# Luolin0826/band

Hardware: AMD Instinct MI355X
Metric: multi-DNN inferences/sec + p99 job latency, 4-model int8 mix @1/2/4/8 GPU (higher is better)
Workload: dtype int8

## Files before the change

### band_amd/_abi.py

```python
import ctypes
import os

_HERE = os.path.dirname(os.path.abspath(__file__))
LIB_PATH = os.path.join(_HERE, "libband_hip%s.so" % (
    "_" + os.environ["BAND_HIP_LIB_VARIANT"] if os.environ.get("BAND_HIP_LIB_VARIANT") else ""))

c_int, c_int32, c_void_p, c_size_t = ctypes.c_int, ctypes.c_int32, ctypes.c_void_p, ctypes.c_size_t


class ConvParams(ctypes.Structure):
    _fields_ = [(n, c_int) for n in (
        "batch", "in_h", "in_w", "in_c", "out_h", "out_w", "out_c", "k_h", "k_w",
        "stride_h", "stride_w", "dil_h", "dil_w", "pad_h", "pad_w", "k_pad", "n_pad", "in_xor")] + [
        (n, c_int32) for n in ("in_zp", "w_zp", "out_zp", "act_min", "act_max")] + [
        (n, c_void_p) for n in ("input", "output", "weights", "bias_eff", "mult", "shift", "residual")] + [
        (n, c_int32) for n in ("add_y_off", "add_r_off", "add_o_off", "add_left_shift", "add_y_mult",
                               "add_y_shift", "add_r_mult", "add_r_shift", "add_o_mult", "add_o_shift",
                               "add_act_min", "add_act_max")] + [("out_table", c_void_p), ("requant_fast", c_int32),
                                                                  ("kernel_hint", c_int32),
                                                                  ("out_img_stride", ctypes.c_int64)]


class ConvGroupedParams(ctypes.Structure):
    _fields_ = [("conv", ConvParams), ("groups", c_int32)]
# ... 62 lines not shown


class LayerNormParams(ctypes.Structure):
    _fields_ = [("rows", ctypes.c_long), ("depth", c_int), ("mean_x", MeanRowsParams), ("mean_d", MeanRowsParams)] + [
        (n, EltwiseParams) for n in ("sqdiff", "add_eps", "mul_gamma", "mul_x", "mul_m", "sub_beta", "add_out")] + [
        ("eps_q", c_int32)] + [(n, c_void_p) for n in ("rsqrt_table", "input", "gamma", "beta", "output")]


LAYERNORM_F32_MAX_DEPTH = 1024


class LayerNormF32Params(ctypes.Structure):
    _fields_ = [("rows", ctypes.c_long), ("depth", c_int), ("eps", ctypes.c_float)] + [
        (n, c_void_p) for n in ("input", "gamma", "beta", "output", "q", "scale", "offset")] + [("asymmetric", c_int)]


class DetectionParams(ctypes.Structure):
    _fields_ = [(n, c_int) for n in ("batch", "num_boxes", "num_classes", "num_classes_with_background",
                                     "max_detections")] + [
        (n, ctypes.c_float) for n in ("score_threshold", "iou_threshold", "scale_y", "scale_x", "scale_h",
                                      "scale_w")] + [
        ("box_type", c_int), ("score_type", c_int), ("box_scale", ctypes.c_float), ("score_scale", ctypes.c_float),
        ("box_zp", c_int32), ("score_zp", c_int32)] + [
        (n, c_void_p) for n in ("box_encodings", "class_scores", "anchors", "out_boxes", "out_classes",
                                "out_scores", "out_num", "scratch")]


class ChainParams(ctypes.Structure):
    _fields_ = [("dw", DwConvParams), ("pw1", ConvParams), ("pw2", ConvParams), ("has_pw2", c_int),
                ("px_blocks", c_int), ("waves", c_int), ("persist", c_int), ("tile", c_int),
                ("tile_blob", c_void_p), ("debug_stamps", c_void_p), ("deep", c_int), ("c_split", c_int),
                ("stage", c_int), ("dense", c_int)]


CONCAT_MAX_INPUTS = 16


class ConcatParams(ctypes.Structure):
    _fields_ = [("n_inputs", c_int), ("outer", ctypes.c_long),
                ("row", ctypes.c_long * CONCAT_MAX_INPUTS), ("input", c_void_p * CONCAT_MAX_INPUTS),
                ("table", c_void_p * CONCAT_MAX_INPUTS), ("output", c_void_p)]


class PadParams(ctypes.Structure):
    _fields_ = [("elem_bytes", c_int), ("in_shape", c_int * 4), ("pad_before", c_int * 4),
                ("pad_after", c_int * 4), ("value", ctypes.c_uint32), ("input", c_void_p), ("output", c_void_p),
                ("mode", c_int32)]


class ResizeNearestParams(ctypes.Structure):
    _fields_ = [(n, c_int) for n in ("batch", "in_h", "in_w", "out_h", "out_w", "row_bytes")] + [
        (n, c_void_p) for n in ("y_index", "x_index", "input", "output")]


class ResizeBilinearParams(ctypes.Structure):
    _fields_ = [(n, c_int) for n in ("batch", "in_h", "in_w", "channels", "out_h", "out_w")] + [
        (n, c_void_p) for n in ("y_tab", "x_tab", "input", "output")]


ARG_I8, ARG_U8, ARG_F32 = 0, 1, 2


class ArgMinMaxParams(ctypes.Structure):
    _fields_ = [(n, ctypes.c_long) for n in ("outer", "axis_len", "inner")] + [
        (n, c_int) for n in ("in_type", "is_min", "out_bytes")] + [("input", c_void_p), ("output", c_void_p)]

# ... 200 lines not shown
    "bh_dynquant_rows_check": (c_int, [ctypes.POINTER(DynQuantParams)]),
    "bh_fc_hybrid": (c_int, [ctypes.POINTER(FcHybridParams), c_void_p]),
    "bh_fc_hybrid_kernel": (ctypes.c_char_p, [ctypes.POINTER(FcHybridParams)]),
    "bh_fc_hybrid_check": (c_int, [ctypes.POINTER(FcHybridParams)]),
    "bh_dynquant_items": (c_int, [ctypes.POINTER(DynQuantItemsParams), c_void_p]),
    "bh_dynquant_items_kernel": (ctypes.c_char_p, [ctypes.POINTER(DynQuantItemsParams)]),
    "bh_dynquant_items_check": (c_int, [ctypes.POINTER(DynQuantItemsParams)]),
    "bh_conv2d_hybrid": (c_int, [ctypes.POINTER(ConvHybridParams), c_void_p]),
    "bh_conv2d_hybrid_kernel": (ctypes.c_char_p, [ctypes.POINTER(ConvHybridParams)]),
    "bh_conv2d_hybrid_check": (c_int, [ctypes.POINTER(ConvHybridParams)]),
    "bh_dwconv2d_hybrid": (c_int, [ctypes.POINTER(ConvHybridParams), c_void_p]),
    "bh_dwconv2d_hybrid_kernel": (ctypes.c_char_p, [ctypes.POINTER(ConvHybridParams)]),
    "bh_dwconv2d_hybrid_check": (c_int, [ctypes.POINTER(ConvHybridParams)]),
    "bh_softmax_i8": (c_int, [ctypes.POINTER(SoftmaxParams), c_void_p]),
    "bh_attention_i8": (c_int, [ctypes.POINTER(AttentionParams), c_void_p]),
    "bh_attention_i8_kernel": (ctypes.c_char_p, [ctypes.POINTER(AttentionParams)]),
    "bh_attention_i8_check": (c_int, [ctypes.POINTER(AttentionParams)]),
    "bh_attention_i8_lds_bytes": (c_size_t, [ctypes.POINTER(AttentionParams)]),
    "bh_zero_insert": (c_int, [ctypes.POINTER(ZeroInsertParams), c_void_p]),
    "bh_conv2d_f32": (c_int, [ctypes.POINTER(ConvF32Params), c_void_p]),
    "bh_conv2d_f32_split": (c_int, [ctypes.POINTER(ConvF32Params)]),
    "bh_fc_f32": (c_int, [ctypes.POINTER(FcF32Params), c_void_p]),
    "bh_eltwise_f32": (c_int, [ctypes.POINTER(EltwiseF32Params), c_void_p]),
    "bh_pool_f32": (c_int, [ctypes.POINTER(PoolF32Params), c_void_p]),
    "bh_unary_f32": (c_int, [c_int, c_void_p, c_void_p, ctypes.c_long, ctypes.c_float, ctypes.c_float, c_void_p]),
    "bh_softmax_f32": (c_int, [c_void_p, c_void_p, ctypes.c_long, c_int, ctypes.c_float, c_void_p]),
    "bh_dwconv2d_i8": (c_int, [ctypes.POINTER(DwConvParams), c_void_p]),
    "bh_fc_i8": (c_int, [ctypes.POINTER(FcParams), c_void_p]),
    "bh_eltwise_i8": (c_int, [ctypes.POINTER(EltwiseParams), c_void_p]),
    "bh_pool_i8": (c_int, [ctypes.POINTER(PoolParams), c_void_p]),
    "bh_irb_i8": (c_int, [ctypes.POINTER(IrbParams), c_void_p]),
    "bh_irb_lds_bytes": (c_size_t, [ctypes.POINTER(IrbParams)]),
    "bh_chain_i8": (c_int, [ctypes.POINTER(ChainParams), c_void_p]),
    "bh_mean": (c_int, [ctypes.POINTER(MeanParams), c_void_p]),
    "bh_mean_rows": (c_int, [ctypes.POINTER(MeanRowsParams), c_void_p]),
    "bh_mean_rows_kernel": (ctypes.c_char_p, [ctypes.POINTER(MeanRowsParams)]),
    "bh_mean_rows_check": (c_int, [ctypes.POINTER(MeanRowsParams)]),
    "bh_layernorm_i8": (c_int, [ctypes.POINTER(LayerNormParams), c_void_p]),
    "bh_layernorm_i8_kernel": (ctypes.c_char_p, [ctypes.POINTER(LayerNormParams)]),
    "bh_layernorm_i8_check": (c_int, [ctypes.POINTER(LayerNormParams)]),
    "bh_layernorm_f32": (c_int, [ctypes.POINTER(LayerNormF32Params), c_void_p]),
    "bh_layernorm_f32_kernel": (ctypes.c_char_p, [ctypes.POINTER(LayerNormF32Params)]),
    "bh_layernorm_f32_check": (c_int, [ctypes.POINTER(LayerNormF32Params)]),
    "bh_detection_scratch_bytes": (c_size_t, [c_int, c_int]),
    "bh_detection_postprocess": (c_int, [ctypes.POINTER(DetectionParams), c_void_p]),
    "bh_chain_lds_bytes": (c_size_t, [ctypes.POINTER(ChainParams)]),
    "bh_chain_tile_lds_bytes": (c_size_t, [ctypes.POINTER(ChainParams)]),
    "bh_chain_tile_launch": (c_int, [ctypes.POINTER(ChainParams), c_void_p]),
    "bh_chain_tile_blob_bytes": (c_size_t, [ctypes.POINTER(ChainParams)]),
    "bh_chain_tile_pack": (c_int, [ctypes.POINTER(ChainParams), c_void_p, c_void_p]),
    "bh_chain_stage_lds_bytes": (c_size_t, [ctypes.POINTER(ChainParams)]),
    "bh_chain_stage_launch": (c_int, [ctypes.POINTER(ChainParams), c_void_p]),
    "bh_chain_dense_lds_bytes": (c_size_t, [ctypes.POINTER(ChainParams)]),
    "bh_chain_dense_launch": (c_int, [ctypes.POINTER(ChainParams), c_void_p]),
    "bh_last_error": (ctypes.c_char_p, []),
}

BACKEND_SYMBOLS = {}

_lib = None
_configured = set()


class BandHipError(RuntimeError):
    pass

# ... 24 lines not shown
```

### band_amd/csrc/backend/hip/fusion.cc

```cpp
#include "backend/hip/chain_form.h"
#include "backend/hip/env.h"
#include "backend/hip/executor_internal.h"
#include <mutex>
#include <optional>
#include <unordered_map>

namespace band {
namespace hip {

using namespace ex;

namespace {
bool LaunchIo(const Launch& l, std::vector<const void*>* rd, std::vector<const void*>* wr) {
  switch (l.kind()) {
    case Launch::kConv:
    case Launch::kConvGrouped:
      *rd = {l.conv().input, l.conv().residual};
      *wr = {l.conv().output};
      return true;
    case Launch::kDwConv:
      *rd = {l.as<bh_dwconv_params>().input};
      *wr = {l.as<bh_dwconv_params>().output};
      return true;
    case Launch::kChain: {
// ... 514 lines not shown
    bh_chain_params& fc = F.Set<Launch::kChain>();
    F.op_index = D.op_index;
    if (form.launches == 0 || !instantiate(form, &fc)) {
      out.push_back(L[i]);
      continue;
    }
    if (fc.tile_blob) sg->consts.push_back(form.launches == 3 ? blob3 : blob2);
    const bool three = form.launches == 3;
    F.out_tensor = three ? P2->out_tensor : P1.out_tensor;
    F.kernel = fc.dense   ? "chain_dense_kernel"
               : fc.stage ? "chain_stage_kernel"
                          : (fc.tile ? "chain_tile_kernel" : "chain_kernel");
    const bh_dwconv_params& dw = fc.dw;
    const bh_conv_params& a = fc.pw1;
    const double px = static_cast<double>(dw.batch) * dw.out_h * dw.out_w;
    F.alg_bytes = static_cast<double>(dw.batch) * dw.in_h * dw.in_w * dw.in_c + 9.0 * dw.out_c + 28.0 * dw.out_c +
                  (a.residual ? px * a.out_c : 0.0) + (a.output ? px * a.out_c : 0.0) +
                  static_cast<double>(a.out_c) * a.in_c + 12.0 * a.out_c;
    F.alg_ops = D.alg_ops + P1.alg_ops;
    if (three) {
      const bh_conv_params& b = fc.pw2;
      F.alg_bytes += px * b.out_c + static_cast<double>(b.out_c) * b.in_c + 12.0 * b.out_c;
      F.alg_ops += P2->alg_ops;
      if (!a.output) sg->fused_tensors.insert(P1.out_tensor);
    }
    out.push_back(F);
    sg->fused_tensors.insert(D.out_tensor);
    i += three ? 2 : 1;
  }
  sg->launches.swap(out);
}

namespace {
void** OutSlot(Launch& l) {
  switch (l.kind()) {
    case Launch::kChain: {
      bh_chain_params& c = l.as<bh_chain_params>();
      return c.has_pw2 ? &c.pw2.output : &c.pw1.output;
    }
    case Launch::kConv:
    case Launch::kConvGrouped: return &l.conv().output;
    case Launch::kDwConv: return &l.as<bh_dwconv_params>().output;
    case Launch::kFc: return &l.as<bh_fc_params>().output;
    case Launch::kEltwise: return &l.as<bh_eltwise_params>().out;
    case Launch::kPool: return &l.as<bh_pool_params>().output;
    case Launch::kIrb: return &l.as<bh_irb_params>().output;
    case Launch::kLutU8: return &l.as<LutArgs>().dst;
    default: return nullptr;
  }
}
const void** TableSlot(Launch& l) {
  switch (l.kind()) {
    case Launch::kConv:
    case Launch::kConvGrouped: return l.conv().residual ? nullptr : &l.conv().out_table;
    case Launch::kDwConv: return &l.as<bh_dwconv_params>().out_table;
    case Launch::kFc: return &l.as<bh_fc_params>().out_table;
    default: return nullptr;
  }
}
}

void HipModelExecutor::FuseGlue(const HipModel& model, PreparedSubgraph* sg) {
  const TflModel& d = model.desc();
  auto private_chain = [&](int t, int to, std::vector<int>* chain) {
    while (t >= 0) {
      if (consumers_[t].size() != 1 || KeptOutside(d, *sg, t)) return false;
// ... 121 lines not shown
```

### band_amd/csrc/backend/hip/launch.h

```cpp
#pragma once

#include <cstddef>
#include <cstdint>
#include <cstdio>
#include <cstdlib>
#include <memory>
#include <type_traits>
#include <utility>
#include <variant>
#include <vector>

#include "backend/hip/cpu_kernels.h"
#include "band_hip_kernels.h"

namespace band {
namespace hip {

struct CopyArgs {
  void* dst;
  const void* src;
  size_t bytes;
};
struct LutArgs {
  const void* src;
// ... 117 lines not shown
      {kEltwiseF32, kIndex<bh_eltwise_f32_params>},
      {kPoolF32, kIndex<bh_pool_f32_params>},
      {kUnaryF32, kIndex<UnaryF32Args>},
      {kSoftmaxF32, kIndex<SoftmaxF32Args>},
      {kResizeBilinearU8, kIndex<bh_resize_bilinear_u8_params>},
      {kDetectionPost, kIndex<CpuDetectionParams>},
      {kMean, kIndex<bh_mean_params>},
      {kMeanRows, kIndex<bh_mean_rows_params>},
      {kConvGroup, kIndex<ConvGroupArgs>},
      {kDetectionGpu, kIndex<bh_detection_params>},
      {kArgMinMax, kIndex<bh_argminmax_params>},
      {kResizeArgMinMax, kIndex<bh_resize_argminmax_params>},
      {kReindex, kIndex<bh_reindex_params>},
      {kConvGrouped, kIndex<bh_conv_grouped_params>},
      {kBatchMatMul, kIndex<bh_batch_matmul_params>},
      {kBatchMatMulF32, kIndex<bh_batch_matmul_params>},
      {kLayerNorm, kIndex<LayerNormArgs>},
      {kAttention, kIndex<bh_attention_params>},
      {kDynQuantRows, kIndex<bh_dynquant_params>},
      {kFcHybrid, kIndex<bh_fc_hybrid_params>},
      {kDynQuantItems, kIndex<bh_dynquant_items_params>},
      {kConvHybrid, kIndex<bh_conv_hybrid_params>},
      {kDwConvHybrid, kIndex<bh_conv_hybrid_params>},
      {kLayerNormF32, kIndex<bh_layernorm_f32_params>},
  };
  template <Kind K>
  using PayloadOf = std::variant_alternative_t<kPayloads[K].index, Payload>;

  int op_index = -1;
  int out_tensor = -1;
  double alg_bytes = 0;
  double alg_ops = 0;
  const char* kernel = "";

  Kind kind() const { return kind_; }

  template <Kind K>
  PayloadOf<K>& Set(PayloadOf<K> p = {}) {
    kind_ = K;
    return payload_.template emplace<PayloadOf<K>>(std::move(p));
  }
  template <class P>
  P& Set(Kind k, P p) {
    if (k < 0 || k >= kNumKinds || kPayloads[k].index != kIndex<P>) Mismatch(k, kIndex<P>);
    kind_ = k;
    return payload_.template emplace<P>(std::move(p));
  }

  template <class P>
  P* get_if() { return std::get_if<P>(&payload_); }
  template <class P>
  const P* get_if() const { return std::get_if<P>(&payload_); }
  template <class P>
  P& as() {
    if (P* p = get_if<P>()) return *p;
    Mismatch(kind_, kIndex<P>);
  }
  template <class P>
  const P& as() const { return const_cast<Launch*>(this)->as<P>(); }

  bh_conv_params* conv_if() {
    if (bh_conv_grouped_params* g = get_if<bh_conv_grouped_params>()) return &g->conv;
    return get_if<bh_conv_params>();
  }
  const bh_conv_params* conv_if() const { return const_cast<Launch*>(this)->conv_if(); }
  bh_conv_params& conv() {
// ... 30 lines not shown
```

### band_amd/csrc/backend/hip/lower.cc

```cpp
#include "backend/hip/executor_internal.h"

namespace band {
namespace hip {

using namespace ex;

namespace {

struct ConvQuant {
  std::vector<int32_t> mult, shift;
  int32_t amin, amax, in_zp, w_zp;
  const int32_t* bias;
};

ConvQuant QuantOf(const TflModel& d, const ConvGeometry& g, const TflTensor& out) {
  const TflTensor& in = d.tensors[g.input];
  const TflTensor& w = d.tensors[g.filter];
  const bool i8 = in.type == DataType::kInt8;
  ConvQuant q;
  ConvMultipliers(Scale(in), w.scale, g.out_c, Scale(out), !i8, &q.mult, &q.shift);
  ActivationRangeQuantized(g.act, Scale(out), Zp(out), i8, &q.amin, &q.amax);
  q.in_zp = Dom(in);
  q.w_zp = i8 ? 0 : Dom(w);
  q.bias = g.bias >= 0 ? reinterpret_cast<const int32_t*>(d.tensors[g.bias].data) : nullptr;
// ... 380 lines not shown
        bh_resize_bilinear_params& p = L->Set<Launch::kResizeBilinear>();
        p.batch = b; p.in_h = ih; p.in_w = iw; p.channels = c; p.out_h = oh; p.out_w = ow;
        p.y_tab = static_cast<const int32_t*>(dt);
        p.x_tab = static_cast<const int32_t*>(dt) + 3 * oh;
        p.input = in_ptr;
        p.output = out_ptr;
        L->kernel = "resize_bilinear_kernel";
      }
      return absl::OkStatus();
    }
    default:
      return absl::InternalError(std::string("no lowering for ") + TflBuiltinName(op.builtin));
  }
}

absl::Status HipModelExecutor::BuildLaunches(const HipModel& model, PreparedSubgraph* sg) {
  sg->launches.clear();
  sg->fused_ops.clear();
  sg->fused_tensors.clear();
  for (int i : sg->ops) {
    if (sg->fused_ops.count(i)) continue;
    RETURN_STATUS_IF(Lower(model, i, sg));
  }
  if (opt_.allow_fusion && opt_.allow_chain && device_flag_ == DeviceFlag::kGPU) FuseChains(model, sg);
  if (opt_.allow_fusion && opt_.allow_irb && device_flag_ == DeviceFlag::kGPU) FuseBlocks(model, sg);
  if (opt_.allow_fusion && opt_.allow_layernorm && device_flag_ == DeviceFlag::kGPU) FuseLayerNorm(model, sg);
  if (opt_.allow_fusion && opt_.allow_layernorm && opt_.fused_layernorm_f32 && device_flag_ == DeviceFlag::kGPU) {
    FuseLayerNormF32(model, sg);
    FoldLayerNormQuant(model, sg);
  }
  if (opt_.allow_fusion && opt_.fused_attention && device_flag_ == DeviceFlag::kGPU) FuseAttention(model, sg);
  if (opt_.allow_fusion) FuseGlue(model, sg);
  if (opt_.allow_fusion && opt_.allow_group && device_flag_ == DeviceFlag::kGPU) RETURN_STATUS_IF(GroupConvs(sg));
  return absl::OkStatus();
}

bool HipModelExecutor::TryFuseResidualAdd(const HipModel& model, int oi, PreparedSubgraph* sg, Launch* L) {
  if (!opt_.allow_fusion || !opt_.allow_add) return false;
  const TflModel& d = model.desc();
  const int t = d.ops[oi].outputs[0];
  if (consumers_[t].size() != 1) return false;
  const int j = consumers_[t][0];
  if (j <= oi || !std::binary_search(sg->ops.begin(), sg->ops.end(), j)) return false;
  const TflOperator& add = d.ops[j];
  if ((add.builtin != kTflAdd && add.builtin != kTflSub) || add.inputs.size() != 2) return false;
  if (!GpuSupports(d, add, nullptr)) return false;
  if (KeptOutside(d, *sg, t)) return false;
  const bool conv_is_first = add.inputs[0] == t;
  const int other = conv_is_first ? add.inputs[1] : add.inputs[0];
  if (other == t) return false;
  if (other < 0 || producer_[other] > oi) return false;
  const TflTensor& tc = d.tensors[t];
  const TflTensor& tr = d.tensors[other];
  const TflTensor& to = d.tensors[add.outputs[0]];
  if (tr.shape != tc.shape || to.shape != tc.shape || tr.type != tc.type || to.type != tc.type) return false;
  void* rptr = nullptr;
  void* optr = nullptr;
  if (!DevicePtr(model, other, sg, &rptr).ok() || !DevicePtr(model, add.outputs[0], sg, &optr).ok()) return false;
  const TflTensor& t1 = d.tensors[add.inputs[0]];
  const TflTensor& t2 = d.tensors[add.inputs[1]];
  const AddParams ap = AddSubParams(Scale(t1), Scale(t2), Scale(to), add.builtin == kTflSub);
  bh_conv_params& p = L->conv();
  p.residual = rptr;
  p.output = optr;
  p.add_left_shift = ap.left_shift;
  p.add_y_off = -Zp(tc);
// ... 791 lines not shown
```

### band_amd/csrc/backend/hip/model_executor.cc

```cpp
#include "backend/hip/model_executor.h"

#include <sys/prctl.h>
#include <time.h>

#include <chrono>
#include <limits>
#include <mutex>
#include <unordered_map>

#include "backend/hip/affinity.h"
#include "backend/hip/completion.h"
#include "backend/hip/env.h"
#include "backend/hip/executor_internal.h"

namespace band {
namespace hip {

using namespace ex;

namespace ex {
thread_local bool t_variant_ctor = false;
}


// ... 7 lines not shown
    stream_ = DeviceRegistry::Get().StreamForWorker(worker_id_);
  } else if (device_flag_ == DeviceFlag::kCPU && !t_variant_ctor) {
    cpu_pool_ = std::make_shared<CpuPool>(num_threads_ > 0 ? num_threads_ : 1, PinnableCpus(thread_affinity_mask_));
  }
  use_graph_ = env::Graph();
  const std::string m(env::Sync());
  sync_mode_ = m == "block"    ? kSyncBlock
               : m == "poll"     ? kSyncPoll
               : m == "poller"   ? kSyncPoller
               : m == "spin"     ? kSyncSpin
                                 : kSyncAdaptive;
  block_sync_ = sync_mode_ == kSyncBlock;
  direct_io_ = env::DirectIo();
  coalesce_max_ = env::Coalesce();
  coalesce_lanes_ = env::CoalesceLanes();
  opt_.Latch(false);
}

void ExecOptions::Latch(bool bound) {
  if (!bound) {
    gpu_detection = env::GpuDetection();
    hybrid_conv = env::HybridConv();
  }
  if (!bound || latched) return;
  latched = true;
  const char* f = env::Fusion();
  if (f[0] == '0') allow_fusion = false;
  if (std::strcmp(f, "noirb") == 0) allow_irb = false;
  if (std::strcmp(f, "noadd") == 0) allow_add = false;
  if (std::strcmp(f, "nochain") == 0) allow_chain = false;
  if (std::strcmp(f, "nogroup") == 0) allow_group = false;
  if (std::strcmp(f, "noargmax") == 0) allow_argmax = false;
  if (std::strcmp(f, "nolayernorm") == 0) allow_layernorm = false;
  if (std::strcmp(f, "forcechain") == 0) forced_chain = ForcedChain::kPlain;
  if (std::strcmp(f, "forcetile") == 0) forced_chain = ForcedChain::kTile;
  if (std::strcmp(f, "forcedeep") == 0) forced_chain = ForcedChain::kDeep;
  if (std::strcmp(f, "forcestage") == 0) forced_chain = ForcedChain::kStage;
  if (std::strcmp(f, "forcedense") == 0) forced_chain = ForcedChain::kDense;
  if (std::strcmp(f, "notile") == 0) no_tile_chain = true;
  if (std::strcmp(f, "nodeep") == 0) no_deep_chain = true;
  if (std::strcmp(f, "nosplit") == 0) no_split_chain = true;
  if (std::strcmp(f, "nostage") == 0) no_stage_chain = true;
  autotune = env::Autotune();
  fused_attention = env::FusedAttention();
  fused_layernorm_f32 = env::FusedLayerNormF32();
}

HipModelExecutor::~HipModelExecutor() {
  if (coalescer_) coalescer_->Leave(this);
  coalescer_.reset();
  job_batches_.clear();
  if (ordinal_ >= 0) {
    bh_set_device(ordinal_);
    if (stream_) bh_stream_sync(stream_);
    for (auto& kv : subgraphs_) DropGraph(kv.second.get());
    if (done_event_) bh_event_destroy(done_event_);
  }
  subgraphs_.clear();
  if (owned_stream_) bh_stream_destroy(owned_stream_);
}

std::unique_ptr<HipModelExecutor> HipModelExecutor::MakeLane() {
  if (device_flag_ != DeviceFlag::kGPU || ordinal_ < 0) return nullptr;
  auto lane = std::make_unique<HipModelExecutor>(model_id_, worker_id_, device_flag_, thread_affinity_mask_,
                                                 num_threads_);
  if (bh_set_device(ordinal_) != 0 || bh_stream_create(&lane->owned_stream_) != 0) return nullptr;
// ... 486 lines not shown
  return std::make_shared<HipTensorView>(m, nullptr);
}

namespace {

struct KindCalls {
  Launch::Kind kind;
  int (*device)(const Launch&, bh_stream_t);
  void (*host)(const Launch&, CpuPool&);
};

template <class F>
struct BlockOf;
template <class R, class P, class... A>
struct BlockOf<R (*)(const P*, A...)> {
  using type = P;
};
template <class R, class P, class... A>
struct BlockOf<R (*)(const P&, A...)> {
  using type = P;
};
template <auto Fn>
int Dev(const Launch& l, bh_stream_t s) {
  return Fn(&l.as<typename BlockOf<decltype(Fn)>::type>(), s);
}
template <auto Fn>
void Host(const Launch& l, CpuPool& pool) {
  const auto& p = l.as<typename BlockOf<decltype(Fn)>::type>();
  if constexpr (std::is_invocable_v<decltype(Fn), decltype(p), CpuPool&>) Fn(p, pool);
  else Fn(p);
}

constexpr KindCalls kCalls[] = {
    {Launch::kConv, Dev<bh_conv2d_i8>, Host<CpuConv>},
    {Launch::kDwConv, Dev<bh_dwconv2d_i8>, Host<CpuDwConv>},
    {Launch::kFc, Dev<bh_fc_i8>, Host<CpuFc>},
    {Launch::kEltwise, Dev<bh_eltwise_i8>, Host<CpuEltwise>},
    {Launch::kPool, Dev<bh_pool_i8>, Host<CpuPool2D>},
    {Launch::kCopy,
     [](const Launch& l, bh_stream_t s) {
       const CopyArgs& c = l.as<CopyArgs>();
       return c.src != c.dst ? bh_copy_d2d(c.dst, c.src, c.bytes, s) : 0;
     },
     [](const Launch& l, CpuPool&) {
       const CopyArgs& c = l.as<CopyArgs>();
       if (c.src != c.dst) std::memmove(c.dst, c.src, c.bytes);
     }},
    {Launch::kIrb, Dev<bh_irb_i8>, nullptr},
    {Launch::kChain, Dev<bh_chain_i8>, nullptr},
    {Launch::kLutU8,
     [](const Launch& l, bh_stream_t s) {
       const LutArgs& a = l.as<LutArgs>();
       return bh_lut_u8(a.src, a.dst, a.count, a.table, s);
     },
     [](const Launch& l, CpuPool& pool) {
       const LutArgs& a = l.as<LutArgs>();
       CpuLutU8(a.src, a.dst, a.count, static_cast<const uint8_t*>(a.table), pool);
     }},
    {Launch::kLutF32,
     [](const Launch& l, bh_stream_t s) {
       const LutArgs& a = l.as<LutArgs>();
       return bh_lut_f32(a.src, a.dst, a.count, static_cast<const float*>(a.table), s);
     },
     [](const Launch& l, CpuPool& pool) {
       const LutArgs& a = l.as<LutArgs>();
       CpuLutF32(a.src, static_cast<float*>(a.dst), a.count, static_cast<const float*>(a.table), pool);
     }},
// ... 401 lines not shown
```

### band_amd/csrc/backend/hip/model_executor.h

```cpp
#pragma once

#include <functional>
#include <map>
#include <memory>
#include <set>
#include <string>
#include <vector>

#include "backend/hip/chain_form.h"
#include "backend/hip/coalescer.h"
#include "backend/hip/cpu_kernels.h"
#include "backend/hip/device.h"
#include "backend/hip/model.h"
#include "backend/hip/tensor.h"
#include "backend/hip/job_batching.h"
#include "backend/hip/launch.h"
#include "backend/hip/lower_args.h"
#include "band/interface/model_executor.h"
#include "band_hip_kernels.h"

namespace band {
namespace hip {

struct LnMatch;
// ... 10 lines not shown
  std::vector<int> ops;
  std::vector<int> inputs, outputs;
  bool model_order_io = false;
  std::map<int, size_t> offset;
  std::shared_ptr<DeviceBlob> arena;
  std::map<int, std::unique_ptr<PinnedBuffer>> host;
  std::set<int> extra_d2h;
  std::set<int> fused_ops;
  std::set<int> fused_tensors;
  std::set<int> no_fuse;
  std::vector<Launch> launches;
  std::vector<std::shared_ptr<DeviceBlob>> consts;
  bh_graph_exec_t graph = nullptr;
  bool io_in_graph = true;
  void* graph_tmpl = nullptr;
  struct IoNode {
    void* node;
    int tensor;
    bool h2d;
  };
  std::vector<IoNode> io_nodes;
  bool io_retargeted = false;
  int runs = 0;
  double wait_us = 0.0;
};

struct ExecOptions {
  bool allow_fusion = true;
  bool allow_irb = true, allow_add = true;
  bool allow_chain = true;
  bool allow_group = true;
  bool allow_argmax = true;
  bool allow_layernorm = true;
  ForcedChain forced_chain = ForcedChain::kNone;
  bool no_tile_chain = false;
  bool no_deep_chain = false;
  bool no_split_chain = false;
  bool no_stage_chain = false;
  bool autotune = true;
  bool gpu_detection = false;
  bool hybrid_conv = false;
  bool fused_attention = false;
  bool fused_layernorm_f32 = false;
  bool latched = false;
  void Latch(bool bound);
};

class HipModelExecutor : public interface::IModelExecutor, public IJobBatching {
 public:
  HipModelExecutor(ModelId model_id, WorkerId worker_id, DeviceFlag device_flag,
                   CpuSet thread_affinity_mask, int num_threads);
  ~HipModelExecutor() override;

  absl::StatusOr<ModelSpec> InvestigateModelSpec(interface::IModel* model) override;
  absl::Status PrepareSubgraph(interface::IModel* model, std::set<int> ops = {},
                               std::set<int> unit_indices = {}) override;
  BackendType GetBackendType() const override { return BackendType::kTfLite; }
  const std::vector<int>& GetInputs(const SubgraphKey& key) const override;
  const std::vector<int>& GetOutputs(const SubgraphKey& key) const override;
  const char* GetInputName(const SubgraphKey& key, int index) const override;
  const char* GetOutputName(const SubgraphKey& key, int index) const override;
  size_t GetNumTensors(const SubgraphKey& key) const override;
  size_t GetNumNodes(const SubgraphKey& key) const override;
  std::shared_ptr<interface::ITensorView> GetTensorView(const SubgraphKey& key, int index) override;
  bool HasSubgraph(const SubgraphKey& key) const override;
  SubgraphKey GetLargestSubgraphKey() const override;
// ... 7 lines not shown
  absl::Status ExecuteJobBatch(const SubgraphKey& key, int n) override;
  absl::Status ExecuteJobBatchDirect(const SubgraphKey& key, int n, const std::vector<const interface::ITensor*>& in,
                                     const std::vector<interface::ITensor*>& out) override;

  void SetUseGraph(bool on) { use_graph_ = on; }
  absl::Status ProfileSubgraph(const SubgraphKey& key, int iters, std::vector<OpTiming>* out,
                               double* floor_us = nullptr);
  absl::Status LaunchKernels(const SubgraphKey& key, std::vector<const char*>* out) const;
  absl::Status JobBatchLaunchKernels(const SubgraphKey& key, int n, std::vector<const char*>* out) const;
  absl::Status TimeSubgraph(const SubgraphKey& key, int iters, double* us);
  int ordinal() const { return ordinal_; }
  const JobCoalescer* coalescer() const { return coalescer_.get(); }

  static bool GpuSupports(const TflModel& model, const TflOperator& op, std::string* why);
  static bool CpuSupports(const TflModel& model, const TflOperator& op, std::string* why);
  bool GpuSupportsHere(const TflModel& model, const TflOperator& op, std::string* why) const;
  bool CpuSupportsHere(const TflModel& model, const TflOperator& op, std::string* why) const;

 private:
  friend class JobCoalescer;
  PreparedSubgraph* Find(const SubgraphKey& key) const;
  absl::Status RunPass(PreparedSubgraph* sg);
  std::unique_ptr<HipModelExecutor> MakeLane();
  absl::Status EnsureMeta(const HipModel& model);
  absl::Status Lower(const HipModel& model, int op_index, PreparedSubgraph* sg);
  absl::Status BuildLaunches(const HipModel& model, PreparedSubgraph* sg);
  bool TryFuseResidualAdd(const HipModel& model, int conv_op, PreparedSubgraph* sg, Launch* l);
  void FuseBlocks(const HipModel& model, PreparedSubgraph* sg);
  bool PackChainTile(bh_chain_params* q, std::shared_ptr<DeviceBlob>* blob);
  bool KeptOutside(const TflModel& d, const PreparedSubgraph& sg, int t) const;
  bool PrivateTensor(const TflModel& d, const PreparedSubgraph& sg, int t, int only_consumer) const;
  bool PrivateTo(const TflModel& d, const PreparedSubgraph& sg, int t, const std::set<int>& ops) const;
  void FuseChains(const HipModel& model, PreparedSubgraph* sg);
  void FuseGlue(const HipModel& model, PreparedSubgraph* sg);
  bool MatchLayerNorm(const TflModel& d, const PreparedSubgraph& sg, const std::vector<Launch>& ls, size_t i,
                      const Launch::Kind kinds[10], LnMatch* n) const;
  void FuseTenOps(const TflModel& d, PreparedSubgraph* sg, const Launch::Kind kinds[10],
                  const std::function<bool(const LnMatch& n, const Launch* l, Launch* F)>& fill);
  void FuseLayerNorm(const HipModel& model, PreparedSubgraph* sg);
  void FuseLayerNormF32(const HipModel& model, PreparedSubgraph* sg);
  void FoldLayerNormQuant(const HipModel& model, PreparedSubgraph* sg);
  void FuseAttention(const HipModel& model, PreparedSubgraph* sg);
  absl::Status GroupConvs(PreparedSubgraph* sg);
  double TimeLaunches(const std::vector<const Launch*>& ls, int iters);
  absl::Status DevicePtr(const HipModel& model, int tensor, PreparedSubgraph* sg, void** ptr);
  absl::Status ConstBlob(const std::string& key, size_t bytes, PreparedSubgraph* sg,
                         const std::function<absl::Status(uint8_t*)>& fill, std::shared_ptr<DeviceBlob>* blob);
  absl::Status UploadConst(const std::string& key, const void* data, size_t bytes, PreparedSubgraph* sg,
                           const void** dev);
  absl::Status LowerConv(const HipModel& model, int op_index, void* in_ptr, void* out_ptr, const std::string& ckey,
                         PreparedSubgraph* sg, Launch* l);
  absl::Status PackedConv(const HipModel& model, int op_index, const ex::ConvGeometry& g, bool flip,
                          const void* in_ptr, void* out_ptr, const std::string& ckey, PreparedSubgraph* sg, Launch* l);
  absl::Status LowerDepthwise(const HipModel& model, int op_index, void* in_ptr, void* out_ptr,
                              const std::string& ckey, PreparedSubgraph* sg, Launch* l);
  absl::Status LowerFc(const HipModel& model, int op_index, void* in_ptr, void* out_ptr, const std::string& ckey,
                       PreparedSubgraph* sg, Launch* l);
  absl::Status LowerFcHybrid(const HipModel& model, int op_index, void* in_ptr, void* out_ptr, const std::string& ckey,
                             PreparedSubgraph* sg, Launch* l);
  absl::Status LowerConvHybrid(const HipModel& model, int op_index, void* in_ptr, void* out_ptr, const std::string& ckey,
                               PreparedSubgraph* sg, Launch* l);
  absl::Status LowerEltwise(const HipModel& model, int op_index, void* in_ptr, void* out_ptr, PreparedSubgraph* sg,
                            Launch* l);
  absl::Status LowerPool(const HipModel& model, int op_index, void* in_ptr, void* out_ptr, Launch* l);
  absl::Status LowerMean(const HipModel& model, int op_index, void* in_ptr, void* out_ptr, Launch* l);
  absl::Status LowerArgMinMax(const HipModel& model, int op_index, void* in_ptr, void* out_ptr, Launch* l);
// ... 70 lines not shown
```

### include/band_hip_kernels.h

```cpp
#ifndef BAND_HIP_KERNELS_H_
#define BAND_HIP_KERNELS_H_

#include <stddef.h>
#include <stdint.h>

#ifdef __cplusplus
extern "C" {
#endif

#define BH_EINVAL (-1)

typedef void* bh_stream_t;
typedef void* bh_graph_exec_t;
typedef void* bh_event_t;

int bh_device_count(int* count);
int bh_set_device(int ordinal);
int bh_get_device(int* ordinal);
int bh_device_arch(int ordinal, char* buf, size_t cap);
int bh_device_pci_bus_id(int ordinal, char* buf, int cap);
int bh_stream_create(bh_stream_t* stream);
int bh_stream_destroy(bh_stream_t stream);
int bh_stream_sync(bh_stream_t stream);
int bh_stream_query(bh_stream_t stream);
// ... 173 lines not shown
  int32_t d_zp, d_act_min, d_act_max;
  const int8_t* proj_w; int proj_k_pad;
  const int32_t* proj_bias_eff; const int32_t* proj_mult; const int32_t* proj_shift;
  int32_t p_zp, p_act_min, p_act_max;
  int has_residual;
  int32_t add_p_off, add_x_off, add_o_off, add_left_shift;
  int32_t add_p_mult, add_p_shift, add_x_mult, add_x_shift, add_o_mult, add_o_shift;
  int32_t add_act_min, add_act_max;
  const void* input;
  void* output;
  void* debug_stamps;
  int32_t requant_fast;
} bh_irb_params;

size_t bh_irb_lds_bytes(const bh_irb_params* p);
int bh_irb_i8(const bh_irb_params* p, bh_stream_t s);

typedef struct bh_chain_params {
  bh_dwconv_params dw;
  bh_conv_params pw1;
  bh_conv_params pw2;
  int has_pw2;
  int px_blocks;
  int waves;
  int persist;
  int tile;
  const void* tile_blob;
  void* debug_stamps;
  int deep;
  int c_split;
  int stage;
  int dense;
} bh_chain_params;

size_t bh_chain_lds_bytes(const bh_chain_params* p);
size_t bh_chain_stage_lds_bytes(const bh_chain_params* p);
int bh_chain_stage_launch(const bh_chain_params* p, bh_stream_t s);
size_t bh_chain_dense_lds_bytes(const bh_chain_params* p);
int bh_chain_dense_launch(const bh_chain_params* p, bh_stream_t s);
size_t bh_chain_tile_lds_bytes(const bh_chain_params* p);
int bh_chain_tile_launch(const bh_chain_params* p, bh_stream_t s);
size_t bh_chain_tile_blob_bytes(const bh_chain_params* p);
int bh_chain_tile_pack(const bh_chain_params* p, void* blob, bh_stream_t s);
int bh_chain_i8(const bh_chain_params* p, bh_stream_t s);

typedef struct bh_mean_params {
  long outer, reduce, inner;
  int type;
  int32_t multiplier, shift, bias;
  const void* input;
  void* output;
} bh_mean_params;
int bh_mean(const bh_mean_params* p, bh_stream_t s);

typedef struct bh_mean_rows_params {
  long rows;
  int depth;
  int type;
  int exact;
  float scale, bias;
  int32_t out_zp;
  const void* input;
  void* output;
} bh_mean_rows_params;
int bh_mean_rows(const bh_mean_rows_params* p, bh_stream_t s);
const char* bh_mean_rows_kernel(const bh_mean_rows_params* p);
// ... 384 lines not shown
```

Measured before the change: 124,200.

## Fuse 1x1 conv with following 3x3 depthwise conv into one LDS-resident kernel

Adds a new HIP kernel that computes a 1x1 int8 pointwise conv via MFMA for whole small images, keeps the requantized result tile in LDS, and runs the 3x3 depthwise conv from LDS before writing only the final output. A fusion pass pairs adjacent conv/dwconv launches whose intermediate tensor is private, autotunes among four tile forms against the unfused pair, and caches the choice. This removes the intermediate tensor's global write and read plus one kernel launch for small spatial maps, at the cost of a BM-limited tiling (whole images per tile) and extra autotune time at preparation.

```diff
diff --git a/band_amd/_abi.py b/band_amd/_abi.py
--- a/band_amd/_abi.py
+++ b/band_amd/_abi.py
@@ -118,6 +118,12 @@
                 ("tile_blob", c_void_p), ("debug_stamps", c_void_p), ("deep", c_int), ("c_split", c_int),
                 ("stage", c_int), ("dense", c_int)]
 
+
+class ConvDwParams(ctypes.Structure):
+    _fields_ = [("pw", ConvParams), ("dw", DwConvParams), ("form", c_int)]
+
+
+CONV_DW_128, CONV_DW_64, CONV_DW_32, CONV_DW_64W8 = 1, 2, 3, 4
 
 CONCAT_MAX_INPUTS = 16
 
@@ -384,6 +390,10 @@
     "bh_irb_i8": (c_int, [ctypes.POINTER(IrbParams), c_void_p]),
     "bh_irb_lds_bytes": (c_size_t, [ctypes.POINTER(IrbParams)]),
     "bh_chain_i8": (c_int, [ctypes.POINTER(ChainParams), c_void_p]),
+    "bh_conv_dw": (c_int, [ctypes.POINTER(ConvDwParams), c_void_p]),
+    "bh_conv_dw_ok": (c_int, [ctypes.POINTER(ConvParams), ctypes.POINTER(DwConvParams)]),
+    "bh_conv_dw_images_per_tile": (c_int, [c_int, c_int]),
+    "bh_conv_dw_kernel": (ctypes.c_char_p, [ctypes.POINTER(ConvDwParams)]),
     "bh_mean": (c_int, [ctypes.POINTER(MeanParams), c_void_p]),
     "bh_mean_rows": (c_int, [ctypes.POINTER(MeanRowsParams), c_void_p]),
     "bh_mean_rows_kernel": (ctypes.c_char_p, [ctypes.POINTER(MeanRowsParams)]),
diff --git a/band_amd/csrc/backend/hip/fusion.cc b/band_amd/csrc/backend/hip/fusion.cc
--- a/band_amd/csrc/backend/hip/fusion.cc
+++ b/band_amd/csrc/backend/hip/fusion.cc
@@ -570,6 +570,69 @@
 }
 
 namespace {
+constexpr int kConvDwTuneVersion = 1;
+}
+
+void HipModelExecutor::FuseConvDw(const HipModel& model, PreparedSubgraph* sg) {
+  const TflModel& d = model.desc();
+  std::vector<Launch> out;
+  const auto& L = sg->launches;
+  for (size_t i = 0; i < L.size(); ++i) {
+    const bool pair = L[i].kind() == Launch::kConv && i + 1 < L.size() && L[i + 1].kind() == Launch::kDwConv &&
+                      bh_conv_dw_ok(&L[i].as<bh_conv_params>(), &L[i + 1].as<bh_dwconv_params>()) != 0 &&
+                      PrivateTensor(d, *sg, L[i].out_tensor, L[i + 1].op_index);
+    if (!pair) {
+      out.push_back(L[i]);
+      continue;
+    }
+    const Launch& P = L[i];
+    const Launch& D = L[i + 1];
+    bh_conv_dw_params q{};
+    q.pw = P.as<bh_conv_params>();
+    q.dw = D.as<bh_dwconv_params>();
+    const int by_shape = bh_conv_dw_ok(&q.pw, &q.dw);
+    char key[256];
+    std::snprintf(key, sizeof(key), "cd%d:%d:%d:%dx%dx%d:%d:s%dd%d:t%d%d", kConvDwTuneVersion, ordinal_,
+                  tune_batch_ > 0 ? tune_batch_ : q.pw.batch, q.pw.in_h, q.pw.in_w, q.pw.in_c, q.pw.out_c,
+                  q.dw.stride_h, q.dw.dil_h, q.pw.out_table ? 1 : 0, q.dw.taps ? 1 : 0);
+    const std::optional<int> cached = opt_.autotune && !opt_.force_conv_dw ? TuneLookup(key) : std::nullopt;
+    int form = 0;
+    if (opt_.force_conv_dw) {
+      form = by_shape;
+    } else if (cached) {
+      form = *cached >= 0 && *cached <= BH_CONV_DW_64W8 ? *cached : 0;
+    } else {
+      Fastest best(opt_.autotune ? TimeLaunches({&P, &D}, 10) : -1.0);
+      const bool measured = best.us > 0;
+      for (int f = BH_CONV_DW_128; measured && f <= BH_CONV_DW_64W8; ++f) {
+        if ((f == BH_CONV_DW_128 && q.pw.out_c <= 64) || (f != BH_CONV_DW_128 && f != BH_CONV_DW_32 && q.pw.out_c <= 32)) continue;
+        q.form = f;
+        Launch F = P;
+        F.conv_dw = std::make_shared<const bh_conv_dw_params>(q);
+        if (best.Offer(TimeLaunches({&F}, 10))) form = f;
+      }
+      if (measured) TuneStore(key, form);
+    }
+    if (form == 0) {
+      out.push_back(L[i]);
+      continue;
+    }
+    q.form = form;
+    Launch F = P;
+    F.conv_dw = std::make_shared<const bh_conv_dw_params>(q);
+    F.out_tensor = D.out_tensor;
+    F.kernel = "conv_dw_kernel";
+    const double mid = static_cast<double>(q.pw.batch) * q.pw.out_h * q.pw.out_w * q.pw.out_c;
+    F.alg_bytes = P.alg_bytes + D.alg_bytes - 2.0 * mid;
+    F.alg_ops = P.alg_ops + D.alg_ops;
+    out.push_back(F);
+    sg->fused_tensors.insert(P.out_tensor);
+    ++i;
+  }
+  sg->launches.swap(out);
+}
+
+namespace {
 void** OutSlot(Launch& l) {
   switch (l.kind()) {
     case Launch::kChain: {
diff --git a/band_amd/csrc/backend/hip/launch.h b/band_amd/csrc/backend/hip/launch.h
--- a/band_amd/csrc/backend/hip/launch.h
+++ b/band_amd/csrc/backend/hip/launch.h
@@ -173,6 +173,7 @@
   double alg_bytes = 0;
   double alg_ops = 0;
   const char* kernel = "";
+  std::shared_ptr<const bh_conv_dw_params> conv_dw;
 
   Kind kind() const { return kind_; }
 
diff --git a/band_amd/csrc/backend/hip/lower.cc b/band_amd/csrc/backend/hip/lower.cc
--- a/band_amd/csrc/backend/hip/lower.cc
+++ b/band_amd/csrc/backend/hip/lower.cc
@@ -436,6 +436,7 @@
   if (opt_.allow_fusion && opt_.fused_attention && device_flag_ == DeviceFlag::kGPU) FuseAttention(model, sg);
   if (opt_.allow_fusion) FuseGlue(model, sg);
   if (opt_.allow_fusion && opt_.allow_group && device_flag_ == DeviceFlag::kGPU) RETURN_STATUS_IF(GroupConvs(sg));
+  if (opt_.allow_fusion && opt_.allow_conv_dw && device_flag_ == DeviceFlag::kGPU) FuseConvDw(model, sg);
   return absl::OkStatus();
 }
 
diff --git a/band_amd/csrc/backend/hip/model_executor.cc b/band_amd/csrc/backend/hip/model_executor.cc
--- a/band_amd/csrc/backend/hip/model_executor.cc
+++ b/band_amd/csrc/backend/hip/model_executor.cc
@@ -63,6 +63,8 @@
   if (std::strcmp(f, "nogroup") == 0) allow_group = false;
   if (std::strcmp(f, "noargmax") == 0) allow_argmax = false;
   if (std::strcmp(f, "nolayernorm") == 0) allow_layernorm = false;
+  if (std::strcmp(f, "noconvdw") == 0) allow_conv_dw = false;
+  if (std::strcmp(f, "forceconvdw") == 0) force_conv_dw = true;
   if (std::strcmp(f, "forcechain") == 0) forced_chain = ForcedChain::kPlain;
   if (std::strcmp(f, "forcetile") == 0) forced_chain = ForcedChain::kTile;
   if (std::strcmp(f, "forcedeep") == 0) forced_chain = ForcedChain::kDeep;
@@ -615,7 +617,11 @@
 }
 
 constexpr KindCalls kCalls[] = {
-    {Launch::kConv, Dev<bh_conv2d_i8>, Host<CpuConv>},
+    {Launch::kConv,
+     [](const Launch& l, bh_stream_t s) {
+       return l.conv_dw ? bh_conv_dw(l.conv_dw.get(), s) : bh_conv2d_i8(&l.as<bh_conv_params>(), s);
+     },
+     Host<CpuConv>},
     {Launch::kDwConv, Dev<bh_dwconv2d_i8>, Host<CpuDwConv>},
     {Launch::kFc, Dev<bh_fc_i8>, Host<CpuFc>},
     {Launch::kEltwise, Dev<bh_eltwise_i8>, Host<CpuEltwise>},
diff --git a/band_amd/csrc/backend/hip/model_executor.h b/band_amd/csrc/backend/hip/model_executor.h
--- a/band_amd/csrc/backend/hip/model_executor.h
+++ b/band_amd/csrc/backend/hip/model_executor.h
@@ -66,6 +66,8 @@
   bool allow_group = true;
   bool allow_argmax = true;
   bool allow_layernorm = true;
+  bool allow_conv_dw = true;
+  bool force_conv_dw = false;
   ForcedChain forced_chain = ForcedChain::kNone;
   bool no_tile_chain = false;
   bool no_deep_chain = false;
@@ -139,6 +141,7 @@
   bool PrivateTensor(const TflModel& d, const PreparedSubgraph& sg, int t, int only_consumer) const;
   bool PrivateTo(const TflModel& d, const PreparedSubgraph& sg, int t, const std::set<int>& ops) const;
   void FuseChains(const HipModel& model, PreparedSubgraph* sg);
+  void FuseConvDw(const HipModel& model, PreparedSubgraph* sg);
   void FuseGlue(const HipModel& model, PreparedSubgraph* sg);
   bool MatchLayerNorm(const TflModel& d, const PreparedSubgraph& sg, const std::vector<Launch>& ls, size_t i,
                       const Launch::Kind kinds[10], LnMatch* n) const;
diff --git a/band_amd/csrc/kernels/conv_dw.hip b/band_amd/csrc/kernels/conv_dw.hip
--- /dev/null
+++ b/band_amd/csrc/kernels/conv_dw.hip
@@ -0,0 +1,312 @@
+#include "common.hpp"
+#include "conv_epilogue.hpp"
+
+namespace bh {
+
+typedef __attribute__((address_space(3))) void lds_void_cd_t;
+
+template <int N>
+__device__ __forceinline__ void cd_wait_vmcnt() {
+  static_assert(N >= 0 && N < 64, "vmcnt range");
+  asm volatile("s_waitcnt vmcnt(%0)" ::"n"(N) : "memory");
+}
+
+struct ConvDwDivs {
+  FastDiv ohw, ow;
+};
+
+constexpr int kConvDwBM = 224;
+
+template <int WM, int WN, int WAVES_M, int WAVES_N, int NB, bool FAST>
+__global__ __launch_bounds__(WAVES_M* WAVES_N * 64) void conv_dw_kernel(bh_conv_params p, bh_dwconv_params q, int M,
+                                                                        int K, int ipt, int gm, int gn, int ksteps,
+                                                                        ConvDwDivs dv, XcdSplit xs) {
+  constexpr int W = WAVES_M * WAVES_N;
+  constexpr int T = W * 64;
+  static_assert(W == 4 || W == 8, "4 or 8 waves per workgroup");
+  static_assert(NB >= 2 && NB <= 4, "LDS ring depth");
+  constexpr int BM = WAVES_M * WM * 16;
+  constexpr int BN = WAVES_N * WN * 16;
+  static_assert(BM == kConvDwBM, "the admission rule's tile height");
+  constexpr int ROWS = BM + BN;
+  constexpr int NI = (ROWS + 16 * W - 1) / (16 * W);
+  constexpr int STAGE = NI * 16 * W * 64;
+  constexpr int D = NB - 1;
+  constexpr int PITCH = BN + 4;
+  static_assert(NB * STAGE <= 64 * 1024, "static LDS");
+  static_assert(BM * PITCH <= NB * STAGE, "the image tile reuses the staging buffers");
+  __shared__ __attribute__((aligned(16))) uint8_t lds[NB * STAGE];
+  const int lane = threadIdx.x & 63;
+  const int wave = threadIdx.x >> 6;
+  int bm, bn;
+  xcd_tile((int)blockIdx.x, (int)gridDim.x, xs, gm, gn, bm, bn);
+  if (bm >= gm) return;
+  const int hw = p.out_h * p.out_w;
+  const int img0 = bm * ipt;
+  const int imgs = min(ipt, p.batch - img0);
+  const int rows = imgs * hw;
+  const int tm0 = img0 * hw;
+  const int tn0 = bn * BN;
+  const int N = p.out_c;
+
+  const uint8_t* src[NI];
+  int kval[NI], goff[NI];
+#pragma unroll
+  for (int j = 0; j < NI; ++j) {
+    const int row = 16 * (wave + W * j) + (lane >> 2);
+    const int g = (lane & 3) ^ ((row >> 2) & 3);
+    goff[j] = 16 * g;
+    if (row < BM) {
+      const int m = min(tm0 + min(row, rows - 1), M - 1);
+      src[j] = (const uint8_t*)p.input + (long)m * K + 16 * g;
+      kval[j] = K - 16 * g;
+    } else {
+      const int n = min(min(tn0 + row - BM, tn0 + BN - 1), p.n_pad - 1);
+      src[j] = (const uint8_t*)p.weights + (long)n * p.k_pad + 16 * g;
+      kval[j] = 0x7fffffff;
+    }
+  }
+  auto stage = [&](int ks) {
+    const int kb = ks * 64;
+    uint8_t* dst = lds + (ks % NB) * STAGE + wave * 1024;
+#pragma unroll
+    for (int j = 0; j < NI; ++j) {
+      const uint8_t* s = kb < kval[j] ? src[j] + kb : src[j] - goff[j];
+      __builtin_amdgcn_global_load_lds((const void*)s, (lds_void_cd_t*)(dst + j * W * 1024), 16, 0, 0);
+    }
+  };
+
+  const int r16 = lane & 15;
+  const int g = lane >> 4;
+  const int chunk = ((g ^ (r16 >> 2)) & 3) << 4;
+  const int wm0 = (wave % WAVES_M) * WM * 16;
+  const int wn0 = (wave / WAVES_M) * WN * 16;
+  v4i acc[WM][WN];
+#pragma unroll
+  for (int i = 0; i < WM; ++i)
+#pragma unroll
+    for (int j = 0; j < WN; ++j) acc[i][j] = (v4i){0, 0, 0, 0};
+
+#pragma unroll
+  for (int d = 0; d < D; ++d)
+    if (d < ksteps) stage(d);
+  for (int ks = 0; ks < ksteps; ++ks) {
+    const int ahead = min(D - 1, ksteps - 1 - ks);
+    if (ahead >= 2) cd_wait_vmcnt<2 * NI>();
+    else if (ahead == 1) cd_wait_vmcnt<NI>();
+    else cd_wait_vmcnt<0>();
+    __builtin_amdgcn_s_barrier();
+    if (ks + D < ksteps) stage(ks + D);
+    const uint8_t* buf = lds + (ks % NB) * STAGE;
+    v4i a[WM], b[WN];
+#pragma unroll
+    for (int i = 0; i < WM; ++i) a[i] = *(const v4i*)(buf + (wm0 + i * 16 + r16) * 64 + chunk);
+#pragma unroll
+    for (int j = 0; j < WN; ++j) b[j] = *(const v4i*)(buf + (BM + wn0 + j * 16 + r16) * 64 + chunk);
+#pragma unroll
+    for (int i = 0; i < WM; ++i)
+#pragma unroll
+      for (int j = 0; j < WN; ++j) acc[i][j] = __builtin_amdgcn_mfma_i32_16x16x64_i8(b[j], a[i], acc[i][j], 0, 0, 0);
+    asm volatile("s_waitcnt lgkmcnt(0)" ::: "memory");
+  }
+  cd_wait_vmcnt<0>();
+  __syncthreads();
+
+  {
+    const uint8_t* tab = (const uint8_t*)p.out_table;
+#pragma unroll
+    for (int j = 0; j < WN; ++j) {
+      const int cl = wn0 + j * 16 + 4 * g;
+      if (tn0 + cl >= N) continue;
+      const Chan4 c = chan4(p, tn0 + cl, N);
+#pragma unroll
+      for (int i = 0; i < WM; ++i) {
+        uint32_t packed = 0;
+#pragma unroll
+        for (int r = 0; r < 4; ++r) {
+          const int32_t v = requant_out<FAST>(acc[i][j][r] + c.be[r], c.q[r], p.out_zp, p.act_min, p.act_max);
+          const uint32_t byte = tab ? tab[(uint8_t)v] : ((uint32_t)v & 0xffu);
+          packed |= byte << (8 * r);
+        }
+        *(uint32_t*)(lds + (wm0 + i * 16 + r16) * PITCH + cl) = packed;
+      }
+    }
+  }
+  __syncthreads();
+
+  constexpr int Q = BN / 4;
+  constexpr int SLOTS = T / Q;
+  const int cl = 4 * ((int)threadIdx.x % Q);
+  const int c0 = tn0 + cl;
+  if (c0 >= N) return;
+  const int ohw = q.out_h * q.out_w;
+  const int total = imgs * ohw;
+  const uint32_t zfill = splat_byte(q.in_zp);
+  const uint8_t* otab = (const uint8_t*)q.out_table;
+  uint8_t* out = (uint8_t*)q.output + (long)img0 * ohw * N + c0;
+  const v4i mm = *(const v4i*)(q.mult + c0);
+  const v4i ss = *(const v4i*)(q.shift + c0);
+  ChanQ cq[4];
+#pragma unroll
+  for (int j = 0; j < 4; ++j) cq[j] = chan_q(mm[j], ss[j], q.out_zp);
+  const bool dot = q.taps != nullptr;
+  v4i tw[4];
+  v4i bias4 = (v4i){0, 0, 0, 0};
+  if (dot) {
+#pragma unroll
+    for (int j = 0; j < 4; ++j) tw[j] = ((const v4i*)q.taps)[c0 + j];
+  } else {
+    bias4 = *(const v4i*)(q.bias + c0);
+  }
+  for (int px = (int)threadIdx.x / Q; px < total; px += SLOTS) {
+    const int img = dv.ohw.div(px);
+    const int pl = px - img * ohw;
+    const int oy = dv.ow.div(pl);
+    const int ox = pl - oy * q.out_w;
+    const int y0 = oy * q.stride_h - q.pad_h;
+    const int x0 = ox * q.stride_w - q.pad_w;
+    const uint8_t* tile = lds + img * hw * PITCH + cl;
+    uint32_t xv[9];
+    bool ok[9];
+#pragma unroll
+    for (int fy = 0; fy < 3; ++fy) {
+#pragma unroll
+      for (int fx = 0; fx < 3; ++fx) {
+        const int tap = fy * 3 + fx;
+        const int y = y0 + fy * q.dil_h;
+        const int x = x0 + fx * q.dil_w;
+        ok[tap] = (unsigned)y < (unsigned)q.in_h && (unsigned)x < (unsigned)q.in_w;
+        xv[tap] = ok[tap] ? *(const uint32_t*)(tile + (y * q.in_w + x) * PITCH) : zfill;
+      }
+    }
+    int32_t v[4];
+    if (dot) {
+      uint32_t Tt[4], U[4];
+      {
+        const uint32_t l01 = __builtin_amdgcn_perm(xv[1], xv[0], 0x05010400u);
+        const uint32_t h01 = __builtin_amdgcn_perm(xv[1], xv[0], 0x07030602u);
+        const uint32_t l23 = __builtin_amdgcn_perm(xv[3], xv[2], 0x05010400u);
+        const uint32_t h23 = __builtin_amdgcn_perm(xv[3], xv[2], 0x07030602u);
+        Tt[0] = __builtin_amdgcn_perm(l23, l01, 0x05040100u);
+        Tt[1] = __builtin_amdgcn_perm(l23, l01, 0x07060302u);
+        Tt[2] = __builtin_amdgcn_perm(h23, h01, 0x05040100u);
+        Tt[3] = __builtin_amdgcn_perm(h23, h01, 0x07060302u);
+      }
+      {
+        const uint32_t l01 = __builtin_amdgcn_perm(xv[5], xv[4], 0x05010400u);
+        const uint32_t h01 = __builtin_amdgcn_perm(xv[5], xv[4], 0x07030602u);
+        const uint32_t l23 = __builtin_amdgcn_perm(xv[7], xv[6], 0x05010400u);
+        const uint32_t h23 = __builtin_amdgcn_perm(xv[7], xv[6], 0x07030602u);
+        U[0] = __builtin_amdgcn_perm(l23, l01, 0x05040100u);
+        U[1] = __builtin_amdgcn_perm(l23, l01, 0x07060302u);
+        U[2] = __builtin_amdgcn_perm(h23, h01, 0x05040100u);
+        U[3] = __builtin_amdgcn_perm(h23, h01, 0x07060302u);
+      }
+#pragma unroll
+      for (int j = 0; j < 4; ++j) {
+        const v4i w = tw[j];
+        int32_t a = __builtin_amdgcn_sdot4((int)Tt[j], w.x, w.w, false);
+        a = __builtin_amdgcn_sdot4((int)U[j], w.y, a, false);
+        a = __builtin_amdgcn_sdot4((int)xv[8], w.z, a, false);
+        if (q.w_zp != 0) {
+          int32_t sx = __builtin_amdgcn_sdot4((int)Tt[j], 0x01010101, 0, false);
+          sx = __builtin_amdgcn_sdot4((int)U[j], 0x01010101, sx, false);
+          sx = __builtin_amdgcn_sdot4((int)xv[8], (int)(1u << (8 * j)), sx, false);
+          a -= q.w_zp * sx;
+        }
+        v[j] = requant_out<FAST>(a, cq[j], q.out_zp, q.act_min, q.act_max);
+      }
+    } else {
+      int32_t a[4] = {bias4[0], bias4[1], bias4[2], bias4[3]};
+#pragma unroll
+      for (int tap = 0; tap < 9; ++tap) {
+        if (!ok[tap]) continue;
+        const uint32_t ww = *(const uint32_t*)(q.weights + tap * N + c0);
+#pragma unroll
+        for (int j = 0; j < 4; ++j) a[j] += (sbyte(xv[tap], j) - q.in_zp) * (sbyte(ww, j) - q.w_zp);
+      }
+#pragma unroll
+      for (int j = 0; j < 4; ++j) v[j] = requant_out<false>(a[j], cq[j], q.out_zp, q.act_min, q.act_max);
+    }
+    uint32_t o = 0;
+#pragma unroll
+    for (int j = 0; j < 4; ++j) o |= (otab ? (uint32_t)otab[(uint8_t)v[j]] : ((uint32_t)v[j] & 0xffu)) << (8 * j);
+    *(uint32_t*)(out + (long)px * N) = o;
+  }
+}
+
+template <int WM, int WN, int WAVES_M, int WAVES_N, int NB>
+static int launch_conv_dw(const bh_conv_params& p, const bh_dwconv_params& q, hipStream_t s) {
+  constexpr int BM = WAVES_M * WM * 16;
+  constexpr int BN = WAVES_N * WN * 16;
+  const int hw = p.out_h * p.out_w;
+  const int ipt = BM / hw;
+  const int M = p.batch * hw;
+  const int K = p.in_c;
+  const int gm = (p.batch + ipt - 1) / ipt, gn = (p.out_c + BN - 1) / BN;
+  const XcdSplit xs = xcd_split((long)M * K, (long)p.out_c * K, gm, gn);
+  ConvDwDivs dv;
+  dv.ohw = FastDiv(q.out_h * q.out_w);
+  dv.ow = FastDiv(q.out_w);
+  if (p.requant_fast && q.requant_fast)
+    BH_LAUNCH((conv_dw_kernel<WM, WN, WAVES_M, WAVES_N, NB, true>), dim3(xcd_grid(xs)), dim3(WAVES_M * WAVES_N * 64), 0,
+              s, p, q, M, K, ipt, gm, gn, (K + 63) / 64, dv, xs);
+  else
+    BH_LAUNCH((conv_dw_kernel<WM, WN, WAVES_M, WAVES_N, NB, false>), dim3(xcd_grid(xs)), dim3(WAVES_M * WAVES_N * 64),
+              0, s, p, q, M, K, ipt, gm, gn, (K + 63) / 64, dv, xs);
+  return bh_check_launch("conv_dw_kernel");
+}
+
+}
+
+extern "C" int bh_conv_dw_images_per_tile(int h, int w) {
+  if (h <= 0 || w <= 0 || (long)h * w > bh::kConvDwBM) return 0;
+  return bh::kConvDwBM / (h * w);
+}
+
+extern "C" int bh_conv_dw_ok(const bh_conv_params* pp, const bh_dwconv_params* qq) {
+  if (!pp || !qq) return 0;
+  const bh_conv_params& p = *pp;
+  const bh_dwconv_params& q = *qq;
+  const int K = p.in_c, N = p.out_c;
+  const bool is1x1 = p.k_h == 1 && p.k_w == 1 && p.pad_h == 0 && p.pad_w == 0 && p.stride_h == 1 && p.stride_w == 1;
+  if (!is1x1 || p.batch <= 0 || p.in_h != p.out_h || p.in_w != p.out_w || K <= 0 || N <= 0) return 0;
+  if (p.in_xor != 0 || p.w_zp != 0 || K % 16 != 0 || N % 4 != 0) return 0;
+  if (p.k_pad < K || p.n_pad < N || (p.k_pad % 64) || (p.n_pad % 64)) return 0;
+  if (!p.input || !p.weights || !p.bias_eff || !p.mult || !p.shift) return 0;
+  if (((uintptr_t)p.input & 15) != 0 || ((uintptr_t)p.weights & 15) != 0) return 0;
+  if ((((uintptr_t)p.bias_eff | (uintptr_t)p.mult | (uintptr_t)p.shift) & 15) != 0) return 0;
+  if (p.residual || p.out_img_stride) return 0;
+  if (bh_conv_dw_images_per_tile(p.out_h, p.out_w) == 0) return 0;
+  if ((long)p.batch * p.out_h * p.out_w * (long)(K > N ? K : N) >= INT32_MAX) return 0;
+  if (q.depth_multiplier != 1 || q.k_h != 3 || q.k_w != 3 || q.in_xor != 0) return 0;
+  if (q.batch != p.batch || q.in_h != p.out_h || q.in_w != p.out_w || q.in_c != N || q.out_c != N) return 0;
+  if (q.input != p.output) return 0;
+  if (q.out_h <= 0 || q.out_w <= 0 || q.stride_h <= 0 || q.stride_w <= 0 || q.dil_h <= 0 || q.dil_w <= 0) return 0;
+  if (q.pad_h < 0 || q.pad_w < 0) return 0;
+  if ((long)q.batch * q.out_h * q.out_w * N >= INT32_MAX) return 0;
+  if (!q.output || ((uintptr_t)q.output & 3) != 0 || !q.mult || !q.shift) return 0;
+  if ((((uintptr_t)q.mult | (uintptr_t)q.shift) & 15) != 0) return 0;
+  if (q.taps ? ((uintptr_t)q.taps & 15) != 0 : (!q.weights || !q.bias || ((uintptr_t)q.bias & 15) != 0 || ((uintptr_t)q.weights & 3) != 0))
+    return 0;
+  return N >= 64 ? BH_CONV_DW_64W8 : BH_CONV_DW_32;
+}
+
+extern "C" const char* bh_conv_dw_kernel(const bh_conv_dw_params* p) {
+  return p && bh_conv_dw_ok(&p->pw, &p->dw) ? "conv_dw_kernel" : "";
+}
+
+extern "C" int bh_conv_dw(const bh_conv_dw_params* pp, bh_stream_t stream) {
+  const int form = pp ? bh_conv_dw_ok(&pp->pw, &pp->dw) : 0;
+  if (!form || pp->form < 0 || pp->form > BH_CONV_DW_64W8) {
+    bh_set_last_error("bh_conv_dw: not a 1x1 conv -> 3x3 depthwise pair this kernel takes (bh_conv_dw_ok)");
+    return BH_EINVAL;
+  }
+  hipStream_t s = (hipStream_t)stream;
+  switch (pp->form ? pp->form : form) {
+    case BH_CONV_DW_128: return bh::launch_conv_dw<7, 2, 2, 4, 2>(pp->pw, pp->dw, s);
+    case BH_CONV_DW_64: return bh::launch_conv_dw<7, 2, 2, 2, 3>(pp->pw, pp->dw, s);
+    case BH_CONV_DW_64W8: return bh::launch_conv_dw<7, 1, 2, 4, 2>(pp->pw, pp->dw, s);
+    default: return bh::launch_conv_dw<7, 1, 2, 2, 3>(pp->pw, pp->dw, s);
+  }
+}
diff --git a/include/band_hip_kernels.h b/include/band_hip_kernels.h
--- a/include/band_hip_kernels.h
+++ b/include/band_hip_kernels.h
@@ -229,6 +229,20 @@
   int stage;
   int dense;
 } bh_chain_params;
+
+typedef struct bh_conv_dw_params {
+  bh_conv_params pw;
+  bh_dwconv_params dw;
+  int form;
+} bh_conv_dw_params;
+#define BH_CONV_DW_128 1
+#define BH_CONV_DW_64 2
+#define BH_CONV_DW_32 3
+#define BH_CONV_DW_64W8 4
+int bh_conv_dw_ok(const bh_conv_params* pw, const bh_dwconv_params* dw);
+int bh_conv_dw_images_per_tile(int h, int w);
+int bh_conv_dw(const bh_conv_dw_params* p, bh_stream_t s);
+const char* bh_conv_dw_kernel(const bh_conv_dw_params* p);
 
 size_t bh_chain_lds_bytes(const bh_chain_params* p);
 size_t bh_chain_stage_lds_bytes(const bh_chain_params* p);
```

New measurement: 124,000. Within noise of the previous version (-0.1%).
